# uiuc-robovision/video-dqn

Hardware: AMD Instinct MI355X
Metric: (s,a,r,s') TD-updates/sec, 224x224 frames, batch 256, 1/2/4/8 MI355X (higher is better)
Workload: dtype bf16; 1 GPU; HabitatDQNMultiAction ResNet-18 extra_capacity, 5 categories x 3 actions, full TD update (online fwd on [s;s'], target fwd on s', Double-DQN target + L2 TD loss, backward, Adam); batch_per_gpu=256, global_batch=256, frame=224x224x3 uint8 (normalise fused), parallelism=dp1, target_update_interval=1000, loss_clip=rect, loss_kind=l2, minibatch_pool=4, frame_pack=at the start of every update

## Files before the change

### video_dqn_amd/csrc/igemm.hip

```cpp
#include <stdlib.h>

#include "common.h"

int vdqn_stem_bf16(const void* t_in, const void* wt, const float* bias, void* pool, void* idx, int n_img, int n_idx_img, hipStream_t st);
int vdqn_launch_win9s(const void* igemm_params, hipStream_t stream);
int vdqn_win9s_supports(int cpk, int has_sib);
int vdqn_launch_win9d(const void* igemm_params, hipStream_t stream);
int vdqn_win9d_supports(int ci, int co, int has_sib, int ci2);
int vdqn_launch_win9u(const void* igemm_params, int mode, hipStream_t stream);

#include "igemm_common.h"

namespace {

template <typename T, int BM, int BN, int MODE, int WN, int NS = 2, bool X3 = false>
__global__ __launch_bounds__(BM * WN, 2) void igemm_kernel(const IgemmParams p) {
  static_assert(!X3 || sizeof(T) == 4, "bf16x3 splits f32 operands");
  constexpr int NT = BM * WN;
  constexpr int RPS = NT / 8;
  constexpr int ESZ = (int)sizeof(T);
  constexpr int KC = 128 / ESZ;
  constexpr int NF = BN / (16 * WN);
  constexpr int CPL = 4 * NF;
  constexpr int BROWS = BN / RPS;
// ... 822 lines not shown

  const int cpk = p.ci / KC;
  int i_cc = 0, i_tap = 0, issued = 0;
  int l_cc = 0, l_tap = 0;
#define VDQN_ISSUE_STEP(BBUF)                                              \
  {                                                                        \
    VDQN_ISSUE_B(BBUF, i_tap * cpk + i_cc)                                 \
    if (i_tap == 0) VDQN_ISSUE_AW(i_cc & 1, i_cc)                          \
    if (++i_tap == 9) {                                                    \
      i_tap = 0;                                                           \
      ++i_cc;                                                              \
    }                                                                      \
    ++issued;                                                              \
  }

  u32x4 fa[2][2][4], fb[2][2][NF];
  const unsigned char* a_rd = sA + (wr * 64 + i16) * 128;
  const unsigned char* b_rd = sB + (wc * (BN / WN) + (i16 >> 2) * CPL + (i16 & 3)) * 128;
  const int bcoff0 = ((g ^ (i16 & 7)) << 4), bcoff1 = (((g + 4) ^ (i16 & 7)) << 4);
  const int zoff = (wrows - 1) * 128 + (g << 4);
#define VDQN_LOAD_FRAGS(SET, BBUF)                                                                                       \
  {                                                                                                                      \
    const int kr_ = (l_tap * 11) >> 5, ks_ = l_tap - 3 * kr_;                                    \
    const int ky_ = MODE == 0 ? kr_ : 2 - kr_, kx_ = MODE == 0 ? ks_ : 2 - ks_;                                          \
    const uint32_t tb_ = (ky_ == 0 ? 1u : 0u) | (ky_ == 2 ? 2u : 0u) | (kx_ == 0 ? 4u : 0u) | (kx_ == 2 ? 8u : 0u);       \
    const uint32_t zm_ = edge16 & (tb_ * 0x1111u);                                                                       \
    const int off_ = W * ky_ + kx_;                                                                                      \
    const int key_ = (i16 + off_) & 7;                                                                                   \
    const int ac0_ = ((g ^ key_) << 4), ac1_ = (((g + 4) ^ key_) << 4);                                                  \
    const unsigned char* w_ = sA + (l_cc & 1) * WBYTES;                                                                  \
    const unsigned char* a_ = a_rd + (l_cc & 1) * WBYTES + off_ * 128;                                                   \
    const unsigned char* b_ = b_rd + (BBUF) * (BN * 128);                                                                \
    _Pragma("unroll") for (int f_ = 0; f_ < 4; ++f_) {                                                                   \
      const bool z_ = ((zm_ >> (4 * f_)) & 15u) != 0u;                                                                   \
      fa[SET][0][f_] = *reinterpret_cast<const u32x4*>(z_ ? w_ + zoff : a_ + f_ * 16 * 128 + ac0_);                      \
      fa[SET][1][f_] = *reinterpret_cast<const u32x4*>(z_ ? w_ + zoff + 64 : a_ + f_ * 16 * 128 + ac1_);                 \
    }                                                                                                                    \
    _Pragma("unroll") for (int j_ = 0; j_ < NF; ++j_) {                                                                  \
      fb[SET][0][j_] = *reinterpret_cast<const u32x4*>(b_ + j_ * 4 * 128 + bcoff0);                                      \
      fb[SET][1][j_] = *reinterpret_cast<const u32x4*>(b_ + j_ * 4 * 128 + bcoff1);                                      \
    }                                                                                                                    \
    if (++l_tap == 9) {                                                                                                  \
      l_tap = 0;                                                                                                         \
      ++l_cc;                                                                                                            \
    }                                                                                                                    \
  }
#define VDQN_MFMA_ALL(SET)                                                                                               \
  _Pragma("unroll") for (int h_ = 0; h_ < 2; ++h_) _Pragma("unroll") for (int f_ = 0; f_ < 4; ++f_)                     \
      _Pragma("unroll") for (int j_ = 0; j_ < NF; ++j_) {                                                                \
    acc[f_][j_] = __builtin_amdgcn_mfma_f32_16x16x32_bf16(__builtin_bit_cast(bf16x8, fb[SET][h_][j_]),                   \
                                                          __builtin_bit_cast(bf16x8, fa[SET][h_][f_]), acc[f_][j_], 0, 0, 0); \
  }
#ifdef VDQN_STAMP
  unsigned long long st_wait = 0, st_bar = 0, st_issue = 0, st_comp = 0, st_t = 0;
  const unsigned long long st_begin = __builtin_amdgcn_s_memtime();
  const unsigned long long st_rt_begin = __builtin_amdgcn_s_memrealtime();
#define VDQN_ST(ACC)                                                     \
  {                                                                      \
    const unsigned long long n_ = __builtin_amdgcn_s_memtime();          \
    ACC += n_ - st_t;                                                    \
    st_t = n_;                                                           \
  }
#else
#define VDQN_ST(ACC)
#endif
#define VDQN_STEP(K, CUR, NXT)                                                                                           \
  {                                                                                                                      \
    VDQN_ST(st_comp)                                                                                                     \
    asm volatile("s_waitcnt vmcnt(0) lgkmcnt(0)" ::: "memory");                                                          \
    VDQN_ST(st_wait)                                                                                                     \
    asm volatile("" : "+v"(fa[CUR][0][0]), "+v"(fa[CUR][0][1]), "+v"(fa[CUR][0][2]), "+v"(fa[CUR][0][3]),                \
                      "+v"(fa[CUR][1][0]), "+v"(fa[CUR][1][1]), "+v"(fa[CUR][1][2]), "+v"(fa[CUR][1][3]));               \
    _Pragma("unroll") for (int j_ = 0; j_ < NF; ++j_) asm volatile("" : "+v"(fb[CUR][0][j_]), "+v"(fb[CUR][1][j_]));     \
    __builtin_amdgcn_s_barrier();                                                                                        \
    VDQN_ST(st_bar)                                                                                                      \
    if (issued < nk) VDQN_ISSUE_STEP((K) & 1)                                                                            \
    VDQN_ST(st_issue)                                                                                                    \
    __builtin_amdgcn_sched_barrier(0);                                                                                   \
    VDQN_LOAD_FRAGS(NXT, ((K) + 1) & 1)  \
    VDQN_MFMA_ALL(CUR)                                                                                                   \
    VDQN_INTERLEAVE(8 + 2 * NF)                                                                                          \
    __builtin_amdgcn_sched_barrier(0);                                                                                   \
  }
  VDQN_ISSUE_STEP(0)
  if (issued < nk) VDQN_ISSUE_STEP(1)
  asm volatile("s_waitcnt vmcnt(0)" ::: "memory");
  __builtin_amdgcn_s_barrier();
  VDQN_LOAD_FRAGS(0, 0)
#ifdef VDQN_STAMP
  st_t = __builtin_amdgcn_s_memtime();
#endif
  for (int k = 0; k < nk; k += 2) {
    VDQN_STEP(k, 0, 1)
    if (k + 1 < nk) VDQN_STEP(k + 1, 1, 0)
  }
  VDQN_ST(st_comp)
#undef VDQN_ST
#undef VDQN_LOAD_FRAGS
#undef VDQN_MFMA_ALL
#undef VDQN_STEP
#undef VDQN_ISSUE_STEP
#undef VDQN_ISSUE_AW
#undef VDQN_ISSUE_B
#undef VDQN_DMA4
#undef VDQN_DMA1
#ifdef VDQN_STAMP
  const unsigned long long st_loop_end = __builtin_amdgcn_s_memtime();
#endif
  igemm_epilogue<T, BM, BN, MODE, WN>(p, acc, smem, m0, n0, tile_m, rows_total, p.howo, W, 0, 0, p.bias);
#ifdef VDQN_STAMP
  if (p.pool_out && tid == 0) {
    asm volatile("s_waitcnt vmcnt(0)" ::: "memory");
    unsigned long long* o = reinterpret_cast<unsigned long long*>(p.pool_out) + (size_t)blockIdx.x * 16;
    o[0] = st_begin; o[1] = st_loop_end; o[2] = __builtin_amdgcn_s_memtime();
    o[3] = st_wait; o[4] = st_bar; o[5] = st_issue; o[6] = st_comp; o[7] = (unsigned long long)nk;
    o[8] = st_rt_begin; o[9] = __builtin_amdgcn_s_memrealtime();
    unsigned hwid_;
    asm volatile("s_getreg_b32 %0, hwreg(HW_REG_HW_ID)" : "=s"(hwid_));
    o[10] = hwid_;
  }
#endif
}

#ifdef VDQN_STAMP
}
void* g_stamp_buffer = nullptr;
namespace {
#endif

template <typename T, int MODE>
int launch_igemm_win9(const IgemmParams& p, hipStream_t stream) {
  const int wrows = (128 + 2 * p.wo + 2 + 1 + 7) & ~7;
  const size_t smem = (size_t)2 * wrows * 128 + 2 * 128 * 128;
  vdqn_ensure_dyn_smem(reinterpret_cast<const void*>(&igemm_win9_kernel<T, MODE>), smem);
  const unsigned grid = (unsigned)(p.tiles_m * p.tiles_n);
  vdqn_prof_begin(MODE == 0 ? "igemm_win<bf16,128,fwd>" : "igemm_win<bf16,128,dgrad>", 2.0 * p.M * p.co * p.ktot,
                  2.0 * ((double)p.n_img * p.hi * p.wi * p.ci + (double)p.co * p.ktot + (double)p.M * p.co * (1 + (p.resid != nullptr) + (p.mask != nullptr))), stream);
#ifdef VDQN_STAMP
  IgemmParams ps = p;
  ps.pool_out = g_stamp_buffer;
  hipLaunchKernelGGL((igemm_win9_kernel<T, MODE>), dim3(grid), dim3(256), smem, stream, ps, wrows, make_fastdiv((uint32_t)p.wo), make_fastdiv((uint32_t)p.howo));
  vdqn_prof_end(stream);
  VDQN_LAUNCH_CHECK();
  return VDQN_OK;
#endif
  hipLaunchKernelGGL((igemm_win9_kernel<T, MODE>), dim3(grid), dim3(256), smem, stream, p, wrows, make_fastdiv((uint32_t)p.wo), make_fastdiv((uint32_t)p.howo));
  vdqn_prof_end(stream);
  VDQN_LAUNCH_CHECK();
  return VDQN_OK;
}

constexpr int kC64WinRows = 248;
constexpr int kC64WinBytes = kC64WinRows * 128;
constexpr int kC64LoadTap = 4;
constexpr int kC64RegTaps = 7;
constexpr int kC64Smem = 2 * kC64WinBytes + 256 + 512 + 256 + (9 - kC64RegTaps) * 8192;

template <int MODE, bool HAS_RES, bool HAS_MSK>
__global__ __launch_bounds__(256, 2) void conv64_kernel(const IgemmParams p, const int n_tiles, const FastDiv d_wo, const FastDiv d_howo) {
  using T = bf16raw;
  extern __shared__ __attribute__((aligned(16))) unsigned char smem[];
  unsigned char* sZ = smem + 2 * kC64WinBytes;
  float* sScratch = reinterpret_cast<float*>(sZ + 256);
  float* sBias = reinterpret_cast<float*>(sZ + 256 + 512);
  unsigned char* sWt = sZ + 256 + 512 + 256;
  const int tid = threadIdx.x, lane = tid & 63, wave = tid >> 6;
  const int wave_u = __builtin_amdgcn_readfirstlane(wave);
  const int wr = wave >> 1, wc = wave & 1;
  const int i16 = lane & 15, g = lane >> 4;
  const int W = p.wo, H = p.ho;
  constexpr int g_first = 0;
  const int g_tiles = n_tiles;
  const int g_blocks = (int)gridDim.x;
  const int g_bid = (int)blockIdx.x;
  const unsigned char* w_src = reinterpret_cast<const unsigned char*>(p.wt);
  const float* bias_src = p.bias;
  if (tid < 16) reinterpret_cast<uint4*>(sZ)[tid] = make_uint4(0, 0, 0, 0);
  if (tid >= 64 && tid < 128) sBias[tid - 64] = bias_src ? bias_src[tid - 64] : 0.f;
  const int io_bytes = (int)((long long)p.M * p.ldo * 2);
  const __amdgpu_buffer_rsrc_t r_out = __builtin_amdgcn_make_buffer_rsrc(p.out, 0, io_bytes, 0x00020000);
  const __amdgpu_buffer_rsrc_t r_res = __builtin_amdgcn_make_buffer_rsrc(const_cast<void*>(p.resid), 0, p.resid ? io_bytes : 0, 0x00020000);
  const __amdgpu_buffer_rsrc_t r_msk = __builtin_amdgcn_make_buffer_rsrc(const_cast<void*>(p.mask), 0, p.mask ? io_bytes : 0, 0x00020000);
  const __amdgpu_buffer_rsrc_t r_cs = __builtin_amdgcn_make_buffer_rsrc(p.colsum_part, 0, p.colsum_part ? (int)((long long)n_tiles * p.ldo * 4) : 0, 0x00020000);
  u32x4 held[4] = {};
  uint32_t held_off[4] = {kOob, kOob, kOob, kOob};
  float held_cs = 0.f;
  uint32_t held_cs_off = kOob;

  u32x4 fw[kC64RegTaps][2][2];
  const int wrow0 = wc * 32 + (i16 >> 2) * 8 + (i16 & 3);
  for (int i = tid; i < (9 - kC64RegTaps) * 512; i += 256) {
    const int tt = i >> 9, r = (i >> 3) & 63, c = i & 7;
    *reinterpret_cast<uint4*>(sWt + tt * 8192 + r * 128 + ((c ^ (r & 7)) << 4)) =
        *reinterpret_cast<const uint4*>(w_src + (size_t)r * (576 * 2) + (kC64RegTaps + tt) * 128 + c * 16);
  }
  {
    const unsigned char* wbase = w_src + (size_t)wrow0 * (576 * 2) + g * 16;
#pragma unroll
    for (int t = 0; t < kC64RegTaps; ++t)
#pragma unroll
      for (int h = 0; h < 2; ++h)
#pragma unroll
        for (int j = 0; j < 2; ++j) fw[t][h][j] = *reinterpret_cast<const u32x4*>(wbase + (size_t)j * 4 * (576 * 2) + t * 128 + h * 64);
  }
  __builtin_amdgcn_s_waitcnt(0x0F70);

  const unsigned long long a_ptr = (unsigned long long)p.in;
  const i32x4 rs_a = {__builtin_amdgcn_readfirstlane((int)(unsigned)a_ptr), __builtin_amdgcn_readfirstlane((int)((a_ptr >> 32) & 0xffff)),
                      __builtin_amdgcn_readfirstlane((int)p.in_bytes), 0x00020000};
  const uint32_t lds_base = (uint32_t)(uintptr_t)(__attribute__((address_space(3))) unsigned char*)smem;
  const uint32_t lds_wave = lds_base + (uint32_t)wave_u * (8 * 128);
  const int lrow = tid >> 3;
  const int lchunk = (tid & 7) ^ (lrow & 7);
  constexpr int PSTR = 32 * 128;

  auto issue_window = [&](int tl, int buf) {
    const int q0 = tl * 128 - W - 1;
    uint32_t vo[8];
#pragma unroll
    for (int i = 0; i < 8; ++i) {
      const int q = q0 + lrow + 32 * i;
      vo[i] = (uint32_t)q * 128u + (uint32_t)(lchunk * 16);
    }
    const uint32_t l0 = lds_wave + (uint32_t)(buf * kC64WinBytes);
#pragma unroll
    for (int q = 0; q < 3; ++q) {
      const uint32_t l_ = l0 + (uint32_t)(2 * q * PSTR);
      asm volatile(
          "s_nop 4\n\t"
          "s_mov_b32 m0, %2\n\ts_nop 0\n\tbuffer_load_dwordx4 %0, %3, 0 offen lds\n\t"
          "s_add_u32 m0, %2, %4\n\ts_nop 0\n\tbuffer_load_dwordx4 %1, %3, 0 offen lds"
          ::"v"(vo[2 * q]), "v"(vo[2 * q + 1]), "s"(l_), "s"(rs_a), "n"(PSTR)
          : "memory", "scc");
    }
    {
      const uint32_t l_ = l0 + (uint32_t)(6 * PSTR);
      asm volatile("s_nop 4\n\ts_mov_b32 m0, %1\n\ts_nop 0\n\tbuffer_load_dwordx4 %0, %2, 0 offen lds" ::"v"(vo[6]), "s"(l_), "s"(rs_a) : "memory");
      if (wave_u < 3) {
        const uint32_t l2_ = l_ + (uint32_t)PSTR;
        asm volatile("s_nop 4\n\ts_mov_b32 m0, %1\n\ts_nop 0\n\tbuffer_load_dwordx4 %0, %2, 0 offen lds" ::"v"(vo[7]), "s"(l2_), "s"(rs_a) : "memory");
      }
    }
  };

  auto issue_window_part = [&](int tl, int buf, int part) {
    const int q0 = tl * 128 - W - 1;
    const uint32_t v0 = (uint32_t)(q0 + lrow + 32 * (2 * part)) * 128u + (uint32_t)(lchunk * 16);
    const uint32_t v1 = v0 + 32u * 128u;
    const uint32_t l_ = lds_wave + (uint32_t)(buf * kC64WinBytes) + (uint32_t)(2 * part * PSTR);
    if (part < 3) {
      asm volatile(
          "s_mov_b32 m0, %2\n\ts_nop 0\n\tbuffer_load_dwordx4 %0, %3, 0 offen lds\n\t"
          "s_add_u32 m0, %2, %4\n\ts_nop 0\n\tbuffer_load_dwordx4 %1, %3, 0 offen lds"
          ::"v"(v0), "v"(v1), "s"(l_), "s"(rs_a), "n"(PSTR)
          : "memory", "scc");
    } else {
      asm volatile("s_mov_b32 m0, %1\n\ts_nop 0\n\tbuffer_load_dwordx4 %0, %2, 0 offen lds" ::"v"(v0), "s"(l_), "s"(rs_a) : "memory");
      if (wave_u < 3) {
        const uint32_t l2_ = l_ + (uint32_t)PSTR;
        asm volatile("s_mov_b32 m0, %1\n\ts_nop 0\n\tbuffer_load_dwordx4 %0, %2, 0 offen lds" ::"v"(v1), "s"(l2_), "s"(rs_a) : "memory");
      }
    }
  };
  (void)issue_window_part;
#ifndef VDQN_C64_SPREAD
#define VDQN_C64_SPREAD 1
#endif
  constexpr bool kSpread = VDQN_C64_SPREAD == 2 || (VDQN_C64_SPREAD == 1 && MODE == 0);
  const uint32_t c64_adv_oh = (uint32_t)((16 / W) % H), c64_adv_ow = (uint32_t)(16 - (16 / W) * W);
  int t = g_bid, buf = 0;
  if (t < g_tiles) issue_window(g_first + (int)xcd_remap((uint32_t)t, (uint32_t)g_tiles), 0);
  for (; t < g_tiles; t += g_blocks, buf ^= 1) {
    const int tl = g_first + (int)xcd_remap((uint32_t)t, (uint32_t)g_tiles);
    const int m0 = tl * 128;
#ifdef VDQN_STAMP
    const unsigned long long st_w0 = __builtin_amdgcn_s_memtime();
#endif
    asm volatile("s_waitcnt vmcnt(0)" ::: "memory");
    __builtin_amdgcn_s_barrier();
#ifdef VDQN_STAMP
    const int st_k = (t - g_bid) / g_blocks;
    unsigned long long* st_row = (p.pool_out && st_k < 16) ? reinterpret_cast<unsigned long long*>(p.pool_out) + ((size_t)blockIdx.x * 16 + st_k) * 8 : nullptr;
    if (st_row && tid == 0) { st_row[0] = st_w0; st_row[1] = __builtin_amdgcn_s_memtime(); }
#endif
    const bool c64_has_nx = t + g_blocks < g_tiles;
    const int c64_tl_nx = c64_has_nx ? g_first + (int)xcd_remap((uint32_t)(t + g_blocks), (uint32_t)g_tiles) : 0;
    if constexpr (!kSpread) {
      if (c64_has_nx) issue_window(c64_tl_nx, buf ^ 1);
    }
#ifdef VDQN_STAMP
    if (st_row && tid == 0) st_row[2] = __builtin_amdgcn_s_memtime();
#endif
#pragma unroll
    for (int f = 0; f < 4; ++f) __builtin_amdgcn_raw_buffer_store_b128(held[f], r_out, (int)held_off[f], 0, 0);
    __builtin_amdgcn_raw_buffer_store_b32(__float_as_uint(held_cs), r_cs, (int)held_cs_off, 0, 0);

    uint32_t edge = 0u;
    {
      const uint32_t m = (uint32_t)(m0 + wr * 64 + i16);
      const uint32_t rem = m - fastdiv(m, d_howo) * d_howo.div;
      uint32_t oh = fastdiv(rem, d_wo), ow = rem - oh * d_wo.div;
      const uint32_t adv_oh = c64_adv_oh, adv_ow = c64_adv_ow;
#pragma unroll
      for (int f = 0; f < 4; ++f) {
        edge |= ((oh == 0 ? 1u : 0u) | (oh == (uint32_t)H - 1 ? 2u : 0u) | (ow == 0 ? 4u : 0u) | (ow == (uint32_t)W - 1 ? 8u : 0u)) << (4 * f);
        ow += adv_ow;
        oh += adv_oh;
        const bool c1 = ow >= (uint32_t)W;
        ow -= c1 ? (uint32_t)W : 0u;
        oh += c1 ? 1u : 0u;
        oh -= oh >= (uint32_t)H ? (uint32_t)H : 0u;
      }
    }
    f32x4 acc[4][2];
#pragma unroll
    for (int f = 0; f < 4; ++f)
#pragma unroll
      for (int j = 0; j < 2; ++j) acc[f][j] = (f32x4){0.f, 0.f, 0.f, 0.f};
    const unsigned char* a_rd = smem + buf * kC64WinBytes + (wr * 64 + i16) * 128;
    const int ncol = wc * 32 + g * 8;
    uint32_t off[4];
#pragma unroll
    for (int f = 0; f < 4; ++f) {
      const int m = m0 + wr * 64 + f * 16 + i16;
      off[f] = m < p.M ? (uint32_t)(m * p.ldo + ncol) * 2u : kOob;
    }
    u32x4 rv[4], mv[4];
    constexpr int NSET = (HAS_RES && HAS_MSK) ? 1 : 2;
    u32x4 fa[NSET][4], wl[NSET][2];
#define VDQN_C64_LOAD(HS, SET)                                                                                              \
  {                                                                                                                         \
    constexpr int tap_ = (HS) >> 1, h_ = (HS) & 1;                                                                          \
    constexpr int kr_ = tap_ / 3, ks_ = tap_ % 3;                                                                           \
    constexpr int ky_ = MODE == 0 ? kr_ : 2 - kr_, kx_ = MODE == 0 ? ks_ : 2 - ks_;                     \
    constexpr uint32_t tapbits_ = (ky_ == 0 ? 1u : 0u) | (ky_ == 2 ? 2u : 0u) | (kx_ == 0 ? 4u : 0u) | (kx_ == 2 ? 8u : 0u); \
    const int off_ = W * ky_ + kx_;                                         \
    const int key_ = (i16 + off_) & 7;                                                                                      \
    const int par_ = ((i16 + off_) & 1) << 7;  \
    const int coff_ = ((g + 4 * h_) ^ key_) << 4;                                                                           \
    const unsigned char* z_rd_ = sZ + par_ + coff_;                       \
    _Pragma("unroll") for (int f_ = 0; f_ < 4; ++f_) {                                                                      \
      const bool z_ = (edge & (tapbits_ << (4 * f_))) != 0u;                                                                \
      fa[SET][f_] = *reinterpret_cast<const u32x4*>(z_ ? z_rd_ : a_rd + (f_ * 16 + off_) * 128 + coff_);                    \
    }                                                                                                                       \
    if constexpr (tap_ >= kC64RegTaps) {                                                                                    \
      _Pragma("unroll") for (int j_ = 0; j_ < 2; ++j_)                                                                      \
          wl[SET][j_] = *reinterpret_cast<const u32x4*>(sWt + (tap_ - kC64RegTaps) * 8192 + (wrow0 + j_ * 4) * 128 +        \
                                                        (((g + 4 * h_) ^ ((wrow0 + j_ * 4) & 7)) << 4));                    \
    }                                                                                                                       \
  }
#define VDQN_C64_MMA(HS, SET)                                                                                               \
  {                                                                                                                         \
    constexpr int tap_ = (HS) >> 1, h_ = (HS) & 1;                                                                          \
    _Pragma("unroll") for (int f_ = 0; f_ < 4; ++f_) _Pragma("unroll") for (int j_ = 0; j_ < 2; ++j_) {                     \
      u32x4 w_;                                                                                                             \
      if constexpr (tap_ < kC64RegTaps) w_ = fw[tap_ < kC64RegTaps ? tap_ : 0][h_][j_];                                     \
      else w_ = wl[SET][j_];                                                                                                \
      acc[f_][j_] = __builtin_amdgcn_mfma_f32_16x16x32_bf16(__builtin_bit_cast(bf16x8, w_), __builtin_bit_cast(bf16x8, fa[SET][f_]), acc[f_][j_], 0, 0, 0); \
    }                                                                                                                       \
  }
#define VDQN_C64_SPREAD_ISSUE(HS)                                                                                           \
    if constexpr (kSpread && ((HS)&3) == 2 && (HS) < 16) {                                                                  \
      if (c64_has_nx) issue_window_part(c64_tl_nx, buf ^ 1, (HS) >> 2);                                                     \
      __builtin_amdgcn_sched_barrier(0);                                                                                    \
    }
#define VDQN_C64_STEP(HS)                                                                                                   \
  {                                                                                                                         \
    __builtin_amdgcn_sched_barrier(0);                                                                                      \
    VDQN_C64_SPREAD_ISSUE(HS)                                                                                               \
    if constexpr ((HS) == 2 * kC64LoadTap) {                                                                                \
      if constexpr (HAS_RES) {                                                                                              \
        _Pragma("unroll") for (int f_ = 0; f_ < 4; ++f_) rv[f_] = __builtin_amdgcn_raw_buffer_load_b128(r_res, (int)off[f_], 0, 0); \
      }                                                                                                                     \
      if constexpr (HAS_MSK) {                                                                                              \
        _Pragma("unroll") for (int f_ = 0; f_ < 4; ++f_) mv[f_] = __builtin_amdgcn_raw_buffer_load_b128(r_msk, (int)off[f_], 0, 0); \
      }                                                                                                                     \
      __builtin_amdgcn_sched_barrier(0);                                                                                    \
    }                                                                                                                       \
    if constexpr (NSET == 2) {                                                                                              \
      if constexpr ((HS) + 1 < 18) VDQN_C64_LOAD((HS) + 1, ((HS) + 1) & 1)                                                  \
      VDQN_C64_MMA(HS, (HS) & 1)                                                                                            \
      _Pragma("unroll") for (int g_ = 0; g_ < 6; ++g_) {                                                                    \
        __builtin_amdgcn_sched_group_barrier(0x008, 1, 0);                                                                  \
        __builtin_amdgcn_sched_group_barrier(0x002, 2, 0);                                                                  \
        __builtin_amdgcn_sched_group_barrier(0x100, 1, 0);                                                                  \
      }                                                                                                                     \
    } else {                                                                                                                \
      if constexpr ((HS) > 0) VDQN_C64_LOAD(HS, 0)                                                                          \
      VDQN_C64_MMA(HS, 0)                                                                                                   \
    }                                                                                                                       \
    __builtin_amdgcn_sched_barrier(0);                                                                                      \
  }
#ifdef VDQN_STAMP
    if (st_row && tid == 0) st_row[3] = __builtin_amdgcn_s_memtime();
#endif
    VDQN_C64_LOAD(0, 0)
    VDQN_C64_STEP(0) VDQN_C64_STEP(1) VDQN_C64_STEP(2) VDQN_C64_STEP(3) VDQN_C64_STEP(4) VDQN_C64_STEP(5)
    VDQN_C64_STEP(6) VDQN_C64_STEP(7) VDQN_C64_STEP(8) VDQN_C64_STEP(9) VDQN_C64_STEP(10) VDQN_C64_STEP(11)
    VDQN_C64_STEP(12) VDQN_C64_STEP(13) VDQN_C64_STEP(14) VDQN_C64_STEP(15) VDQN_C64_STEP(16) VDQN_C64_STEP(17)
#undef VDQN_C64_STEP
#undef VDQN_C64_SPREAD_ISSUE
#undef VDQN_C64_MMA
#undef VDQN_C64_LOAD
#ifdef VDQN_STAMP
    if (st_row && tid == 0) { asm volatile("s_nop 0" ::"v"(acc[3][1][3])); st_row[4] = __builtin_amdgcn_s_memtime(); }
#endif
    {
      float bv[8];
      *reinterpret_cast<float4*>(bv) = *reinterpret_cast<const float4*>(sBias + ncol);
      *reinterpret_cast<float4*>(bv + 4) = *reinterpret_cast<const float4*>(sBias + ncol + 4);
      float cs[8];
#pragma unroll
      for (int e = 0; e < 8; ++e) cs[e] = 0.f;
#pragma unroll
      for (int f = 0; f < 4; ++f) {
        float v[8];
#pragma unroll
        for (int j = 0; j < 2; ++j)
#pragma unroll
          for (int r = 0; r < 4; ++r) v[j * 4 + r] = acc[f][j][r] + bv[j * 4 + r];
        if constexpr (HAS_RES) {
          const bf16raw* pr = reinterpret_cast<const bf16raw*>(&rv[f]);
#pragma unroll
          for (int e = 0; e < 8; ++e) v[e] += bf16_to_f32(pr[e]);
        }
        if (p.relu) {
#pragma unroll
          for (int e = 0; e < 8; ++e) v[e] = fmaxf(v[e], 0.f);
        }
        if constexpr (HAS_MSK) {
          const bf16raw* pm = reinterpret_cast<const bf16raw*>(&mv[f]);
#pragma unroll
          for (int e = 0; e < 8; ++e) v[e] = (bf16_to_f32(pm[e]) > 0.f) ? v[e] : 0.f;
        }
        bf16raw ov[8];
#pragma unroll
        for (int e = 0; e < 8; ++e) ov[e] = f32_to_bf16(v[e]);
        if constexpr (MODE == 1) {
          const float live = off[f] != kOob ? 1.f : 0.f;
#pragma unroll
          for (int e = 0; e < 8; ++e) cs[e] += live * bf16_to_f32(ov[e]);
        }
        held[f] = *reinterpret_cast<const u32x4*>(ov);
        held_off[f] = off[f];
      }
      if (MODE == 1 && p.colsum_part) {
#pragma unroll
        for (int e = 0; e < 8; ++e) {
          float t_ = cs[e];
          t_ += __shfl_xor(t_, 1, 64);
          t_ += __shfl_xor(t_, 2, 64);
          t_ += __shfl_xor(t_, 4, 64);
          t_ += __shfl_xor(t_, 8, 64);
          cs[e] = t_;
        }
        if (i16 == 0) {
#pragma unroll
          for (int e = 0; e < 8; ++e) sScratch[wr * 64 + ncol + e] = cs[e];
        }
        asm volatile("s_waitcnt lgkmcnt(0)" ::: "memory");
        __builtin_amdgcn_s_barrier();
        if (tid < 64) {
          held_cs = sScratch[tid] + sScratch[64 + tid];
          held_cs_off = (uint32_t)(tl * p.ldo + tid) * 4u;
        }
      }
    }
#ifdef VDQN_STAMP
    if (st_row && tid == 0) st_row[5] = __builtin_amdgcn_s_memtime();
#endif
  }
#pragma unroll
  for (int f = 0; f < 4; ++f) __builtin_amdgcn_raw_buffer_store_b128(held[f], r_out, (int)held_off[f], 0, 0);
  __builtin_amdgcn_raw_buffer_store_b32(__float_as_uint(held_cs), r_cs, (int)held_cs_off, 0, 0);
}

template <int MODE>
int launch_conv64(const IgemmParams& p, hipStream_t stream) {
  const bool has_res = p.resid != nullptr, has_msk = p.mask != nullptr;
  auto kern = has_res ? (has_msk ? &conv64_kernel<MODE, true, true> : &conv64_kernel<MODE, true, false>)
                      : (has_msk ? &conv64_kernel<MODE, false, true> : &conv64_kernel<MODE, false, false>);
  vdqn_ensure_dyn_smem(reinterpret_cast<const void*>(kern), (size_t)kC64Smem);
  const int n_cu = vdqn_num_cus();
  const int n_tiles = (p.M + 127) / 128;
  int grid = n_tiles < 2 * n_cu ? n_tiles : 2 * n_cu;
  vdqn_prof_begin(MODE == 0 ? "conv64<bf16,fwd>" : "conv64<bf16,dgrad>", 2.0 * p.M * p.co * p.ktot,
                  2.0 * ((double)p.n_img * p.hi * p.wi * p.ci + (double)p.co * p.ktot + (double)p.M * p.co * (1 + (p.resid != nullptr) + (p.mask != nullptr))), stream);
#ifdef VDQN_STAMP
  IgemmParams ps = p;
  ps.pool_out = g_stamp_buffer;
  hipLaunchKernelGGL(kern, dim3(grid), dim3(256), kC64Smem, stream, ps, n_tiles, make_fastdiv((uint32_t)p.wo), make_fastdiv((uint32_t)p.howo));
#else
  hipLaunchKernelGGL(kern, dim3(grid), dim3(256), kC64Smem, stream, p, n_tiles, make_fastdiv((uint32_t)p.wo), make_fastdiv((uint32_t)p.howo));
#endif
  vdqn_prof_end(stream);
  VDQN_LAUNCH_CHECK();
  return VDQN_OK;
}

template <typename T, int BM, int BN, int MODE, int NS = 2, bool X3 = false>
int launch_igemm(const IgemmParams& p, hipStream_t stream) {
  constexpr int WN = (BM == 256 && BN == 64) ? 1 : 2;
  const size_t smem = NS * (BM + BN) * 128;
  vdqn_ensure_dyn_smem(reinterpret_cast<const void*>(&igemm_kernel<T, BM, BN, MODE, WN, NS, X3>), (size_t)smem);
  const unsigned grid = (unsigned)(p.tiles_m * p.tiles_n);
  const double esz = sizeof(T);
  static const char* const kTag[3][4][3] = {{{"igemm<bf16,64,fwd>", "igemm<bf16,64,dgrad>", "igemm<bf16,64,dgrad_s2>"},
                                             {"igemm<bf16,128,fwd>", "igemm<bf16,128,dgrad>", "igemm<bf16,128,dgrad_s2>"},
                                             {"igemm<bf16,256x64,fwd>", "igemm<bf16,256x64,dgrad>", "igemm<bf16,256x64,dgrad_s2>"},
                                             {"igemm<bf16,256x128,fwd>", "igemm<bf16,256x128,dgrad>", "igemm<bf16,256x128,dgrad_s2>"}},
                                            {{"igemm<f32,64,fwd>", "igemm<f32,64,dgrad>", "igemm<f32,64,dgrad_s2>"},
                                             {"igemm<f32,128,fwd>", "igemm<f32,128,dgrad>", "igemm<f32,128,dgrad_s2>"},
                                             {"igemm<f32,256x64,fwd>", "igemm<f32,256x64,dgrad>", "igemm<f32,256x64,dgrad_s2>"},
                                             {"igemm<f32,256x128,fwd>", "igemm<f32,256x128,dgrad>", "igemm<f32,256x128,dgrad_s2>"}},
                                            {{"igemm<bf16x3,64,fwd>", "igemm<bf16x3,64,dgrad>", "igemm<bf16x3,64,dgrad_s2>"},
                                             {"igemm<bf16x3,128,fwd>", "igemm<bf16x3,128,dgrad>", "igemm<bf16x3,128,dgrad_s2>"},
                                             {"igemm<bf16x3,256x64,fwd>", "igemm<bf16x3,256x64,dgrad>", "igemm<bf16x3,256x64,dgrad_s2>"},
                                             {"igemm<bf16x3,256x128,fwd>", "igemm<bf16x3,256x128,dgrad>", "igemm<bf16x3,256x128,dgrad_s2>"}}};
  if constexpr (MODE == 3)
    vdqn_prof_begin(sizeof(T) == 2 ? "stem_conv_pool<bf16>" : (X3 ? "stem_conv_pool<bf16x3>" : "stem_conv_pool<f32>"), 2.0 * p.n_img * 112 * 112 * 64 * 147,
                    esz * ((double)p.n_img * 115 * 115 * 16 + 64.0 * 256 + (double)p.n_img * 56 * 56 * 64) + (double)p.n_img * 56 * 56 * 64, stream);
  else
    vdqn_prof_begin(kTag[sizeof(T) == 2 ? 0 : (X3 ? 2 : 1)][BM == 256 ? (BN == 128 ? 3 : 2) : (BN == 128 ? 1 : 0)][MODE],
                    2.0 * p.M * p.co * p.ktot,
                    esz * ((double)p.n_img * p.hi * p.wi * p.ci + (double)p.co * p.ktot + (double)p.M * p.co * (1 + (p.resid != nullptr) + (p.mask != nullptr))),
                    stream);
  hipLaunchKernelGGL((igemm_kernel<T, BM, BN, MODE, WN, NS, X3>), dim3(grid), dim3(BM * WN), smem, stream, p);
  vdqn_prof_end(stream);
  VDQN_LAUNCH_CHECK();
  return VDQN_OK;
}

template <typename T, int BM, int BN, bool X3 = false>
int launch_mode(const IgemmParams& p, int mode, hipStream_t st) {
  if constexpr (BM == 128) {
    static const bool deep_on = !getenv("VDQN_IGEMM_DEEP") || atoi(getenv("VDQN_IGEMM_DEEP")) != 0;
    if (mode == 0 && deep_on && p.tiles_m * p.tiles_n <= 256 && p.nk >= 8) return launch_igemm<T, BM, BN, 0, 4, X3>(p, st);
  }
  if (mode == 0) return launch_igemm<T, BM, BN, 0, 2, X3>(p, st);
  if (mode == 1) return launch_igemm<T, BM, BN, 1, 2, X3>(p, st);
  if constexpr (BM == 128) return launch_igemm<T, BM, BN, 2, 2, X3>(p, st);
  return VDQN_ERR_INVALID;
}

}

#ifdef VDQN_STAMP
extern "C" void vdqn_debug_stamp_buffer(void* p) { g_stamp_buffer = p; }
#endif

extern "C" int vdqn_conv2d(const vdqn_conv_args* a, void* stream) {
  VDQN_CHECK(a != nullptr, "vdqn_conv2d: null args");
  VDQN_CHECK(a != nullptr, "vdqn_conv2d: null args");
  VDQN_CHECK(a->dtype == VDQN_F32 || a->dtype == VDQN_BF16 || a->dtype == VDQN_F32X3, "vdqn_conv2d: bad dtype %d", a->dtype);
  const int esz = a->dtype == VDQN_BF16 ? 2 : 4;
  const bool x3 = a->dtype == VDQN_F32X3;
  const int kc = 128 / esz;
  VDQN_CHECK(a->in && a->wt && (a->out || a->out_f32), "vdqn_conv2d: null tensor");
  VDQN_CHECK(a->ci > 0 && a->ci % kc == 0, "vdqn_conv2d: ci=%d must be a multiple of %d", a->ci, kc);
  VDQN_CHECK(a->stride == 1 || a->stride == 2, "vdqn_conv2d: stride %d unsupported", a->stride);
  VDQN_CHECK(a->mode == 0 || a->mode == 1, "vdqn_conv2d: bad mode %d", a->mode);
  VDQN_CHECK(a->n_img > 0 && a->ho > 0 && a->wo > 0 && a->co > 0 && a->ldo >= a->co, "vdqn_conv2d: bad dims");
  VDQN_CHECK((int64_t)a->n_img * a->ho * a->wo < (1ll << 31), "vdqn_conv2d: too many output pixels");
  VDQN_CHECK((a->pix_stride * esz) % 16 == 0 && (((uintptr_t)a->in | (uintptr_t)a->wt) & 15) == 0, "vdqn_conv2d: in/wt must be 16-byte aligned");
  IgemmParams p;
  p.in = a->in; p.wt = a->wt; p.bias = a->bias; p.resid = a->resid; p.mask = a->mask; p.out = a->out; p.out_f32 = a->out_f32; p.colsum_part = a->colsum_part;
  p.pool_out = nullptr; p.pool_idx = nullptr;
  p.in2 = nullptr; p.wt2 = nullptr; p.bias2 = nullptr; p.out2 = nullptr;
  p.co2 = p.ldo2 = p.relu2 = p.ci2 = p.wt2_bytes = 0;
  static const int no_lean = [] { const char* e = getenv("VDQN_LEAN_EPILOGUE"); return (e && e[0] == '0') ? 1 : 0; }();
  p.no_lean = no_lean;
  p.n_img = a->n_img; p.hi = a->hi; p.wi = a->wi; p.ci = a->ci; p.pix_stride = a->pix_stride;
  p.ho = a->ho; p.wo = a->wo; p.co = a->co; p.ldo = a->ldo; p.r = a->r; p.s = a->s; p.stride = a->stride; p.pad = a->pad;
  p.relu = a->relu;
  p.M = a->n_img * a->ho * a->wo;
  p.howo = a->ho * a->wo;
  p.ktot = a->r * a->s * a->ci;
  p.nk = p.ktot / kc;
  const int bn = (a->co % 128 == 0) ? 128 : 64;
  p.tiles_m = (p.M + 127) / 128;
  memset(p.cls_tile0, 0, sizeof(p.cls_tile0));
  p.cls_h[0] = p.cls_h[1] = p.cls_w[0] = p.cls_w[1] = 0;
  p.cls_interleave = 0;
  if (a->mode == 1 && a->stride == 2) {
    p.cls_h[0] = (a->ho + 1) / 2; p.cls_h[1] = a->ho / 2;
    p.cls_w[0] = (a->wo + 1) / 2; p.cls_w[1] = a->wo / 2;
    for (int c = 0; c < 4; ++c) p.cls_tile0[c + 1] = p.cls_tile0[c] + (a->n_img * p.cls_h[c >> 1] * p.cls_w[c & 1] + 127) / 128;
    p.tiles_m = p.cls_tile0[4];
    static const int inter = [] { const char* e = getenv("VDQN_DGRAD_S2_INTERLEAVE"); return e ? atoi(e) : 1; }();
    p.cls_interleave = inter && p.cls_h[0] == p.cls_h[1] && p.cls_w[0] == p.cls_w[1];
  }
  p.tiles_n = (a->co + bn - 1) / bn;
  p.tiles_n1 = p.tiles_n;
  const bool has_sib = a->wt2 != nullptr;
  if (has_sib) {
    VDQN_CHECK(a->r == 3 && a->s == 3 && a->stride == 2 && a->pad == 1, "vdqn_conv2d: a sibling 1x1 needs a 3x3 / stride-2 / pad-1 call");
    VDQN_CHECK((((uintptr_t)a->wt2) & 15) == 0, "vdqn_conv2d: wt2 must be 16-byte aligned");
    if (a->mode == 0) {
      VDQN_CHECK(a->out2 && a->co2 > 0 && a->ldo2 >= a->co2 && a->co2 % bn == 0 && bn == 128 && !a->out_f32 && !a->colsum_part,
                 "vdqn_conv2d: fused sibling (forward) needs out2, co2 a multiple of the 128-column tile, no f32 copy / column sums");
      VDQN_CHECK(((a->ldo2 * esz) % 16 == 0) && ((((uintptr_t)a->out2) & 15) == 0) && (a->ldo2 % 8 == 0), "vdqn_conv2d: out2 must be 16-byte aligned rows");
      p.wt2 = a->wt2; p.bias2 = a->bias2; p.out2 = a->out2; p.co2 = a->co2; p.ldo2 = a->ldo2; p.relu2 = a->relu2;
      p.wt2_bytes = (int)((long long)a->co2 * a->ci * esz);
      p.tiles_n = p.tiles_n1 + a->co2 / bn;
    } else {
      VDQN_CHECK(a->in2 && a->ci2 > 0 && a->ci2 % kc == 0 && a->ci2 <= a->pix_stride && (((uintptr_t)a->in2) & 15) == 0,
                 "vdqn_conv2d: fused sibling (data gradient) needs in2 with ci2 (a multiple of %d) channels in pixels of pix_stride elems", kc);
      p.in2 = a->in2; p.wt2 = a->wt2; p.ci2 = a->ci2;
      p.wt2_bytes = (int)((long long)p.tiles_n * bn * a->ci2 * esz);
    }
  }
  p.in_bytes = (long long)a->n_img * a->hi * a->wi * a->pix_stride * esz;
  const long long wtb = (long long)p.tiles_n * bn * p.ktot * esz;
  VDQN_CHECK(wtb < 0x7fffffffLL, "vdqn_conv2d: weight tensor too large");
  p.wt_bytes = (int)wtb;
  const long long img_bytes = (long long)a->hi * a->wi * a->pix_stride * esz;
  const long long span_imgs = 128 / (p.howo > 0 ? p.howo : 1) + 2;
  VDQN_CHECK(span_imgs * img_bytes < 0x7fffffffLL, "vdqn_conv2d: image too large for one tile's gather window");
  const uintptr_t al = (uintptr_t)a->out | (uintptr_t)a->out_f32 | (uintptr_t)a->resid | (uintptr_t)a->mask;
  p.vec_ok = ((a->ldo * esz) % 16 == 0) && ((al & 15) == 0) && (a->ldo % 8 == 0);
  const int mode = a->mode == 0 ? 0 : (a->stride == 2 ? 2 : 1);
  hipStream_t st = (hipStream_t)stream;
  if (mode != 2) {
    const int sk = vdqn_skinny_kind(a);
    if (sk) return vdqn_launch_skinny(&p, sk, st);
  }
  static const int use_c64 = [] { const char* e = getenv("VDQN_CONV64"); return e ? atoi(e) : 1; }();
  if (use_c64 && a->dtype == VDQN_BF16 && a->r == 3 && a->s == 3 && a->stride == 1 && a->pad == 1 && mode != 2 && a->ci == 64 && a->co == 64 &&
      a->pix_stride == 64 && a->hi == a->ho && a->wi == a->wo && a->wo >= 2 && a->wo <= 56 && p.in_bytes < 0x7fffffffLL && (long long)p.M * 128 < 0x7fffffffLL &&
      a->out && !a->out_f32 && p.vec_ok && (long long)p.M * a->ldo * 2 < 0x7fffffffLL && (mode == 1 || !a->colsum_part)) {
    return mode == 0 ? launch_conv64<0>(p, st) : launch_conv64<1>(p, st);
  }
  static const int use_win = [] { const char* e = getenv("VDQN_IGEMM_WINDOW"); return e ? atoi(e) : 1; }();
  if (use_win && a->r == 3 && a->s == 3 && a->stride == 1 && a->pad == 1 && mode != 2 && a->pix_stride == a->ci && a->wo >= 2) {
    if (a->dtype == VDQN_BF16) {
      if (bn == 128 && use_win != 2 && a->wo <= 28 && a->hi == a->ho && a->wi == a->wo && p.in_bytes < 0x7fffffffLL) {
        static const int unrolled = [] { const char* e = getenv("VDQN_WIN9_UNROLLED"); return e ? atoi(e) : 1; }();
        if (unrolled && a->ci % 128 == 0) {
          return vdqn_launch_win9u(&p, mode, st);
        }
        return mode == 0 ? launch_igemm_win9<bf16raw, 0>(p, st) : launch_igemm_win9<bf16raw, 1>(p, st);
      }
      if (bn == 128) return mode == 0 ? launch_igemm_win<bf16raw, 128, 0>(p, st) : launch_igemm_win<bf16raw, 128, 1>(p, st);
      return mode == 0 ? launch_igemm_win<bf16raw, 64, 0>(p, st) : launch_igemm_win<bf16raw, 64, 1>(p, st);
    }
    if (x3) {
// ... 64 lines not shown
```

Baseline: 41390 tuples/s.

## Add contiguous tile walk with sliding LDS window and packed bf16 epilogue in conv64

Adds an optional 'walk' mode where each block processes a contiguous run of tiles and reuses the overlapping window rows in a sliding LDS buffer, loading only the new 128 rows per step instead of the full 248-row window. The default walk stays 0, so the strided schedule is kept unless overridden through a debug hook. The epilogue is also rewritten to use packed f32x2 bias add, bf16x2 conversion, integer-max ReLU and bitmask masking, and it drops the per-row OOB offsets in favour of a base offset plus stride. That epilogue change runs by default. It relies on the buffer resource clamping to handle rows past M, and the larger LDS reservation could affect occupancy.

Result: slower. 40860 tuples/s (-1.3%).

```diff
diff --git a/video_dqn_amd/csrc/igemm.hip b/video_dqn_amd/csrc/igemm.hip
--- a/video_dqn_amd/csrc/igemm.hip
+++ b/video_dqn_amd/csrc/igemm.hip
@@ -998,15 +998,20 @@
 
 constexpr int kC64WinRows = 248;
 constexpr int kC64WinBytes = kC64WinRows * 128;
+constexpr int kC64RunTiles = 3;
+constexpr int kC64BufRows = kC64WinRows + (kC64RunTiles - 1) * 128;
 constexpr int kC64LoadTap = 4;
 constexpr int kC64RegTaps = 7;
-constexpr int kC64Smem = 2 * kC64WinBytes + 256 + 512 + 256 + (9 - kC64RegTaps) * 8192;
+constexpr int kC64FixedBytes = 256 + 512 + 256 + (9 - kC64RegTaps) * 8192;
+constexpr int kC64Smem = kC64FixedBytes + kC64BufRows * 128;
+constexpr int kC64SmemWalk0 = kC64FixedBytes + 2 * kC64WinBytes;
 
 template <int MODE, bool HAS_RES, bool HAS_MSK>
-__global__ __launch_bounds__(256, 2) void conv64_kernel(const IgemmParams p, const int n_tiles, const FastDiv d_wo, const FastDiv d_howo) {
+__global__ __launch_bounds__(256, 2) void conv64_kernel(const IgemmParams p, const int n_tiles, const FastDiv d_wo, const FastDiv d_howo, const int walk) {
   using T = bf16raw;
   extern __shared__ __attribute__((aligned(16))) unsigned char smem[];
-  unsigned char* sZ = smem + 2 * kC64WinBytes;
+  unsigned char* sZ = smem;
+  unsigned char* sWin = smem + kC64FixedBytes;
   float* sScratch = reinterpret_cast<float*>(sZ + 256);
   float* sBias = reinterpret_cast<float*>(sZ + 256 + 512);
   unsigned char* sWt = sZ + 256 + 512 + 256;
@@ -1029,7 +1034,8 @@
   const __amdgpu_buffer_rsrc_t r_msk = __builtin_amdgcn_make_buffer_rsrc(const_cast<void*>(p.mask), 0, p.mask ? io_bytes : 0, 0x00020000);
   const __amdgpu_buffer_rsrc_t r_cs = __builtin_amdgcn_make_buffer_rsrc(p.colsum_part, 0, p.colsum_part ? (int)((long long)n_tiles * p.ldo * 4) : 0, 0x00020000);
   u32x4 held[4] = {};
-  uint32_t held_off[4] = {kOob, kOob, kOob, kOob};
+  uint32_t held_off = kOob;
+  const uint32_t c64_ostr = (uint32_t)(16 * p.ldo * 2);
   float held_cs = 0.f;
   uint32_t held_cs_off = kOob;
 
@@ -1054,23 +1060,23 @@
   const unsigned long long a_ptr = (unsigned long long)p.in;
   const i32x4 rs_a = {__builtin_amdgcn_readfirstlane((int)(unsigned)a_ptr), __builtin_amdgcn_readfirstlane((int)((a_ptr >> 32) & 0xffff)),
                       __builtin_amdgcn_readfirstlane((int)p.in_bytes), 0x00020000};
-  const uint32_t lds_base = (uint32_t)(uintptr_t)(__attribute__((address_space(3))) unsigned char*)smem;
+  const uint32_t lds_base = (uint32_t)(uintptr_t)(__attribute__((address_space(3))) unsigned char*)sWin;
   const uint32_t lds_wave = lds_base + (uint32_t)wave_u * (8 * 128);
   const int lrow = tid >> 3;
   const int lchunk = (tid & 7) ^ (lrow & 7);
   constexpr int PSTR = 32 * 128;
 
-  auto issue_window = [&](int tl, int buf) {
-    const int q0 = tl * 128 - W - 1;
+  auto issue_window = [&](int q0, uint32_t lds_off, bool incr) {
     uint32_t vo[8];
 #pragma unroll
     for (int i = 0; i < 8; ++i) {
       const int q = q0 + lrow + 32 * i;
       vo[i] = (uint32_t)q * 128u + (uint32_t)(lchunk * 16);
     }
-    const uint32_t l0 = lds_wave + (uint32_t)(buf * kC64WinBytes);
+    const uint32_t l0 = lds_wave + lds_off;
 #pragma unroll
     for (int q = 0; q < 3; ++q) {
+      if (q == 2 && incr) break;
       const uint32_t l_ = l0 + (uint32_t)(2 * q * PSTR);
       asm volatile(
           "s_nop 4\n\t"
@@ -1079,7 +1085,7 @@
           ::"v"(vo[2 * q]), "v"(vo[2 * q + 1]), "s"(l_), "s"(rs_a), "n"(PSTR)
           : "memory", "scc");
     }
-    {
+    if (!incr) {
       const uint32_t l_ = l0 + (uint32_t)(6 * PSTR);
       asm volatile("s_nop 4\n\ts_mov_b32 m0, %1\n\ts_nop 0\n\tbuffer_load_dwordx4 %0, %2, 0 offen lds" ::"v"(vo[6]), "s"(l_), "s"(rs_a) : "memory");
       if (wave_u < 3) {
@@ -1089,11 +1095,16 @@
     }
   };
 
-  auto issue_window_part = [&](int tl, int buf, int part) {
-    const int q0 = tl * 128 - W - 1;
+  auto issue_window_part = [&](int q0, uint32_t lds_off, bool incr, int part) {
+    if (incr) {
+      const uint32_t v0 = (uint32_t)(q0 + lrow + 32 * part) * 128u + (uint32_t)(lchunk * 16);
+      const uint32_t l_ = lds_wave + lds_off + (uint32_t)(part * PSTR);
+      asm volatile("s_mov_b32 m0, %1\n\ts_nop 0\n\tbuffer_load_dwordx4 %0, %2, 0 offen lds" ::"v"(v0), "s"(l_), "s"(rs_a) : "memory");
+      return;
+    }
     const uint32_t v0 = (uint32_t)(q0 + lrow + 32 * (2 * part)) * 128u + (uint32_t)(lchunk * 16);
     const uint32_t v1 = v0 + 32u * 128u;
-    const uint32_t l_ = lds_wave + (uint32_t)(buf * kC64WinBytes) + (uint32_t)(2 * part * PSTR);
+    const uint32_t l_ = lds_wave + lds_off + (uint32_t)(2 * part * PSTR);
     if (part < 3) {
       asm volatile(
           "s_mov_b32 m0, %2\n\ts_nop 0\n\tbuffer_load_dwordx4 %0, %3, 0 offen lds\n\t"
@@ -1114,10 +1125,24 @@
 #endif
   constexpr bool kSpread = VDQN_C64_SPREAD == 2 || (VDQN_C64_SPREAD == 1 && MODE == 0);
   const uint32_t c64_adv_oh = (uint32_t)((16 / W) % H), c64_adv_ow = (uint32_t)(16 - (16 / W) * W);
-  int t = g_bid, buf = 0;
-  if (t < g_tiles) issue_window(g_first + (int)xcd_remap((uint32_t)t, (uint32_t)g_tiles), 0);
-  for (; t < g_tiles; t += g_blocks, buf ^= 1) {
-    const int tl = g_first + (int)xcd_remap((uint32_t)t, (uint32_t)g_tiles);
+  int t, t_end;
+  if (walk == 0) {
+    t = g_bid, t_end = g_tiles;
+  } else {
+    const int lb = (int)xcd_remap((uint32_t)g_bid, (uint32_t)g_blocks), base = g_tiles / g_blocks, extra = g_tiles - base * g_blocks;
+    t = lb * base + (lb < extra ? lb : extra);
+    t_end = t + base + (lb < extra ? 1 : 0);
+  }
+  t = __builtin_amdgcn_readfirstlane(t);
+  t_end = __builtin_amdgcn_readfirstlane(t_end);
+  uint32_t rd_off = 0u;
+#ifdef VDQN_STAMP
+  int st_k = 0;
+#endif
+  if (t < t_end) issue_window((walk == 0 ? (int)xcd_remap((uint32_t)t, (uint32_t)g_tiles) : t) * 128 - W - 1, 0u, false);
+  for (; t < t_end; t += (walk == 0 ? g_blocks : 1)) {
+    const int c64_step = walk == 0 ? g_blocks : 1;
+    const int tl = g_first + (walk == 0 ? (int)xcd_remap((uint32_t)t, (uint32_t)g_tiles) : t);
     const int m0 = tl * 128;
 #ifdef VDQN_STAMP
     const unsigned long long st_w0 = __builtin_amdgcn_s_memtime();
@@ -1125,20 +1150,23 @@
     asm volatile("s_waitcnt vmcnt(0)" ::: "memory");
     __builtin_amdgcn_s_barrier();
 #ifdef VDQN_STAMP
-    const int st_k = (t - g_bid) / g_blocks;
     unsigned long long* st_row = (p.pool_out && st_k < 16) ? reinterpret_cast<unsigned long long*>(p.pool_out) + ((size_t)blockIdx.x * 16 + st_k) * 8 : nullptr;
     if (st_row && tid == 0) { st_row[0] = st_w0; st_row[1] = __builtin_amdgcn_s_memtime(); }
 #endif
-    const bool c64_has_nx = t + g_blocks < g_tiles;
-    const int c64_tl_nx = c64_has_nx ? g_first + (int)xcd_remap((uint32_t)(t + g_blocks), (uint32_t)g_tiles) : 0;
+    const bool c64_has_nx = t + c64_step < t_end;
+    const int c64_tl_nx = walk == 0 ? (c64_has_nx ? g_first + (int)xcd_remap((uint32_t)(t + c64_step), (uint32_t)g_tiles) : 0) : tl + 1;
+    const bool c64_incr = walk != 0 && rd_off < (uint32_t)((kC64RunTiles - 1) * 128 * 128);
+    const uint32_t c64_rd_nx = walk == 0 ? (uint32_t)kC64WinBytes - rd_off : (c64_incr ? rd_off + 128u * 128u : 0u);
+    const uint32_t c64_nx = c64_has_nx ? (c64_incr ? (rd_off + (uint32_t)kC64WinBytes) | 1u : c64_rd_nx) : 2u;
+    const int c64_q0_nx = c64_tl_nx * 128 - W - 1 + (c64_incr ? kC64WinRows - 128 : 0);
     if constexpr (!kSpread) {
-      if (c64_has_nx) issue_window(c64_tl_nx, buf ^ 1);
+      if (c64_nx != 2u) issue_window(c64_q0_nx, c64_nx & ~1u, (c64_nx & 1u) != 0u);
     }
 #ifdef VDQN_STAMP
     if (st_row && tid == 0) st_row[2] = __builtin_amdgcn_s_memtime();
 #endif
 #pragma unroll
-    for (int f = 0; f < 4; ++f) __builtin_amdgcn_raw_buffer_store_b128(held[f], r_out, (int)held_off[f], 0, 0);
+    for (int f = 0; f < 4; ++f) __builtin_amdgcn_raw_buffer_store_b128(held[f], r_out, (int)(held_off + (uint32_t)f * c64_ostr), 0, 0);
     __builtin_amdgcn_raw_buffer_store_b32(__float_as_uint(held_cs), r_cs, (int)held_cs_off, 0, 0);
 
     uint32_t edge = 0u;
@@ -1163,14 +1191,9 @@
     for (int f = 0; f < 4; ++f)
 #pragma unroll
       for (int j = 0; j < 2; ++j) acc[f][j] = (f32x4){0.f, 0.f, 0.f, 0.f};
-    const unsigned char* a_rd = smem + buf * kC64WinBytes + (wr * 64 + i16) * 128;
+    const unsigned char* a_rd = sWin + rd_off + (wr * 64 + i16) * 128;
     const int ncol = wc * 32 + g * 8;
-    uint32_t off[4];
-#pragma unroll
-    for (int f = 0; f < 4; ++f) {
-      const int m = m0 + wr * 64 + f * 16 + i16;
-      off[f] = m < p.M ? (uint32_t)(m * p.ldo + ncol) * 2u : kOob;
-    }
+    const uint32_t off0 = (uint32_t)((m0 + wr * 64 + i16) * p.ldo + ncol) * 2u;
     u32x4 rv[4], mv[4];
     constexpr int NSET = (HAS_RES && HAS_MSK) ? 1 : 2;
     u32x4 fa[NSET][4], wl[NSET][2];
@@ -1207,7 +1230,7 @@
   }
 #define VDQN_C64_SPREAD_ISSUE(HS)                                                                                           \
     if constexpr (kSpread && ((HS)&3) == 2 && (HS) < 16) {                                                                  \
-      if (c64_has_nx) issue_window_part(c64_tl_nx, buf ^ 1, (HS) >> 2);                                                     \
+      if (c64_nx != 2u) issue_window_part(c64_q0_nx, c64_nx & ~1u, (c64_nx & 1u) != 0u, (HS) >> 2);                                                  \
       __builtin_amdgcn_sched_barrier(0);                                                                                    \
     }
 #define VDQN_C64_STEP(HS)                                                                                                   \
@@ -1216,10 +1239,10 @@
     VDQN_C64_SPREAD_ISSUE(HS)                                                                                               \
     if constexpr ((HS) == 2 * kC64LoadTap) {                                                                                \
       if constexpr (HAS_RES) {                                                                                              \
-        _Pragma("unroll") for (int f_ = 0; f_ < 4; ++f_) rv[f_] = __builtin_amdgcn_raw_buffer_load_b128(r_res, (int)off[f_], 0, 0); \
+        _Pragma("unroll") for (int f_ = 0; f_ < 4; ++f_) rv[f_] = __builtin_amdgcn_raw_buffer_load_b128(r_res, (int)(off0 + (uint32_t)f_ * c64_ostr), 0, 0); \
       }                                                                                                                     \
       if constexpr (HAS_MSK) {                                                                                              \
-        _Pragma("unroll") for (int f_ = 0; f_ < 4; ++f_) mv[f_] = __builtin_amdgcn_raw_buffer_load_b128(r_msk, (int)off[f_], 0, 0); \
+        _Pragma("unroll") for (int f_ = 0; f_ < 4; ++f_) mv[f_] = __builtin_amdgcn_raw_buffer_load_b128(r_msk, (int)(off0 + (uint32_t)f_ * c64_ostr), 0, 0); \
       }                                                                                                                     \
       __builtin_amdgcn_sched_barrier(0);                                                                                    \
     }                                                                                                                       \
@@ -1252,44 +1275,43 @@
     if (st_row && tid == 0) { asm volatile("s_nop 0" ::"v"(acc[3][1][3])); st_row[4] = __builtin_amdgcn_s_memtime(); }
 #endif
     {
-      float bv[8];
-      *reinterpret_cast<float4*>(bv) = *reinterpret_cast<const float4*>(sBias + ncol);
-      *reinterpret_cast<float4*>(bv + 4) = *reinterpret_cast<const float4*>(sBias + ncol + 4);
+      typedef float f32x2_ __attribute__((ext_vector_type(2)));
+      typedef __bf16 bf16x2_ __attribute__((ext_vector_type(2)));
+      typedef short s16x2_ __attribute__((ext_vector_type(2)));
+      f32x2_ bv[4];
+#pragma unroll
+      for (int e = 0; e < 4; ++e) bv[e] = *reinterpret_cast<const f32x2_*>(sBias + ncol + 2 * e);
+      const short relu_lo_ = p.relu ? (short)0 : (short)-32768;
+      const s16x2_ relu_lo = {relu_lo_, relu_lo_};
       float cs[8];
 #pragma unroll
       for (int e = 0; e < 8; ++e) cs[e] = 0.f;
 #pragma unroll
       for (int f = 0; f < 4; ++f) {
-        float v[8];
-#pragma unroll
-        for (int j = 0; j < 2; ++j)
-#pragma unroll
-          for (int r = 0; r < 4; ++r) v[j * 4 + r] = acc[f][j][r] + bv[j * 4 + r];
-        if constexpr (HAS_RES) {
-          const bf16raw* pr = reinterpret_cast<const bf16raw*>(&rv[f]);
-#pragma unroll
-          for (int e = 0; e < 8; ++e) v[e] += bf16_to_f32(pr[e]);
+        u32x4 ov;
+#pragma unroll
+        for (int e = 0; e < 4; ++e) {
+          f32x2_ v = (f32x2_){acc[f][e >> 1][(e & 1) * 2], acc[f][e >> 1][(e & 1) * 2 + 1]} + bv[e];
+          if constexpr (HAS_RES) v += (f32x2_){__uint_as_float(rv[f][e] << 16), __uint_as_float(rv[f][e] & 0xffff0000u)};
+          s16x2_ o = __builtin_bit_cast(s16x2_, __builtin_convertvector(v, bf16x2_));
+          o = __builtin_elementwise_max(o, relu_lo);
+          if constexpr (HAS_MSK) {
+            const s16x2_ m = __builtin_elementwise_max(__builtin_bit_cast(s16x2_, mv[f][e]), (s16x2_){0, 0});
+            o &= ((s16x2_){0, 0} - m) >> (s16x2_){15, 15};
+          }
+          ov[e] = __builtin_bit_cast(uint32_t, o);
         }
-        if (p.relu) {
-#pragma unroll
-          for (int e = 0; e < 8; ++e) v[e] = fmaxf(v[e], 0.f);
+        if constexpr (MODE == 1) {
+          const float live = m0 + wr * 64 + f * 16 + i16 < p.M ? 1.f : 0.f;
+#pragma unroll
+          for (int e = 0; e < 4; ++e) {
+            cs[2 * e] += live * __uint_as_float(ov[e] << 16);
+            cs[2 * e + 1] += live * __uint_as_float(ov[e] & 0xffff0000u);
+          }
         }
-        if constexpr (HAS_MSK) {
-          const bf16raw* pm = reinterpret_cast<const bf16raw*>(&mv[f]);
-#pragma unroll
-          for (int e = 0; e < 8; ++e) v[e] = (bf16_to_f32(pm[e]) > 0.f) ? v[e] : 0.f;
-        }
-        bf16raw ov[8];
-#pragma unroll
-        for (int e = 0; e < 8; ++e) ov[e] = f32_to_bf16(v[e]);
-        if constexpr (MODE == 1) {
-          const float live = off[f] != kOob ? 1.f : 0.f;
-#pragma unroll
-          for (int e = 0; e < 8; ++e) cs[e] += live * bf16_to_f32(ov[e]);
-        }
-        held[f] = *reinterpret_cast<const u32x4*>(ov);
-        held_off[f] = off[f];
+        held[f] = ov;
       }
+      held_off = off0;
       if (MODE == 1 && p.colsum_part) {
 #pragma unroll
         for (int e = 0; e < 8; ++e) {
@@ -1315,29 +1337,41 @@
 #ifdef VDQN_STAMP
     if (st_row && tid == 0) st_row[5] = __builtin_amdgcn_s_memtime();
 #endif
-  }
-#pragma unroll
-  for (int f = 0; f < 4; ++f) __builtin_amdgcn_raw_buffer_store_b128(held[f], r_out, (int)held_off[f], 0, 0);
+    rd_off = c64_rd_nx;
+#ifdef VDQN_STAMP
+    ++st_k;
+#endif
+  }
+#pragma unroll
+  for (int f = 0; f < 4; ++f) __builtin_amdgcn_raw_buffer_store_b128(held[f], r_out, (int)(held_off + (uint32_t)f * c64_ostr), 0, 0);
   __builtin_amdgcn_raw_buffer_store_b32(__float_as_uint(held_cs), r_cs, (int)held_cs_off, 0, 0);
 }
+
+constexpr int kC64DefaultWalk = 0;
+static int g_conv64_walk_override = -1;
+}
+extern "C" void vdqn_debug_set_conv64_walk(int v) { g_conv64_walk_override = v; }
+namespace {
 
 template <int MODE>
 int launch_conv64(const IgemmParams& p, hipStream_t stream) {
   const bool has_res = p.resid != nullptr, has_msk = p.mask != nullptr;
   auto kern = has_res ? (has_msk ? &conv64_kernel<MODE, true, true> : &conv64_kernel<MODE, true, false>)
                       : (has_msk ? &conv64_kernel<MODE, false, true> : &conv64_kernel<MODE, false, false>);
-  vdqn_ensure_dyn_smem(reinterpret_cast<const void*>(kern), (size_t)kC64Smem);
   const int n_cu = vdqn_num_cus();
   const int n_tiles = (p.M + 127) / 128;
   int grid = n_tiles < 2 * n_cu ? n_tiles : 2 * n_cu;
+  const int walk = g_conv64_walk_override >= 0 ? g_conv64_walk_override : kC64DefaultWalk;
+  const size_t smem = walk == 0 ? kC64SmemWalk0 : kC64Smem;
+  vdqn_ensure_dyn_smem(reinterpret_cast<const void*>(kern), (size_t)kC64Smem);
   vdqn_prof_begin(MODE == 0 ? "conv64<bf16,fwd>" : "conv64<bf16,dgrad>", 2.0 * p.M * p.co * p.ktot,
                   2.0 * ((double)p.n_img * p.hi * p.wi * p.ci + (double)p.co * p.ktot + (double)p.M * p.co * (1 + (p.resid != nullptr) + (p.mask != nullptr))), stream);
 #ifdef VDQN_STAMP
   IgemmParams ps = p;
   ps.pool_out = g_stamp_buffer;
-  hipLaunchKernelGGL(kern, dim3(grid), dim3(256), kC64Smem, stream, ps, n_tiles, make_fastdiv((uint32_t)p.wo), make_fastdiv((uint32_t)p.howo));
+  hipLaunchKernelGGL(kern, dim3(grid), dim3(256), smem, stream, ps, n_tiles, make_fastdiv((uint32_t)p.wo), make_fastdiv((uint32_t)p.howo), walk);
 #else
-  hipLaunchKernelGGL(kern, dim3(grid), dim3(256), kC64Smem, stream, p, n_tiles, make_fastdiv((uint32_t)p.wo), make_fastdiv((uint32_t)p.howo));
+  hipLaunchKernelGGL(kern, dim3(grid), dim3(256), smem, stream, p, n_tiles, make_fastdiv((uint32_t)p.wo), make_fastdiv((uint32_t)p.howo), walk);
 #endif
   vdqn_prof_end(stream);
   VDQN_LAUNCH_CHECK();
```
